# PRBonn/OverlapNet

Hardware: NVIDIA H100
Metric: scan-pairs/sec (overlap+yaw) at 64x900 (higher is better)
Workload: dtype f16

## Files before the change

### overlapnet_b200/csrc/network_tc.cu

```cuda
#include "common.cuh"
#include "hopper.cuh"

#include <cuda_fp16.h>
#include <stddef.h>
#include <stdlib.h>

namespace ovn {

using namespace hopper;

constexpr int WF = 360;
constexpr int CF = 128;
constexpr int S15 = 15;
constexpr int NB = 24;
constexpr int PAIR_ROWS = NB * NB;
constexpr int K4_PITCH = CF;

struct TcState {
  Buffer<__half> w1p;
  Buffer<__half> w2p;
  Buffer<__half> w3p;
  Buffer<float> b2eff;
  Buffer<__half> wres[kMaxLegLayers];
  Buffer<__half> actp[2];
// ... 368 lines not shown
            wgmma_commit();
            if (kk == 1 && sl + 1 < K4_GROUP) rv = *reinterpret_cast<const uint4*>(rp[(sl + 1) & 1] + (sl + 1) * K4_PITCH);
            wgmma_wait<1>();
          }
        wgmma_wait<0>();
        S.w1.release(gi);
      }
      S.right.release(ui);
      if (jb == NB - 1 || u == u_end - 1) S.left.release(pi - 1);
      if (!S.o1s.wait_free(ui)) { atomicExch(err, kErrDeltaO1Consumer); goto done; }
#pragma unroll
      for (int tt = 0; tt < 2; ++tt)
#pragma unroll
        for (int h = 0; h < 2; ++h) {
          if (rows[tt][h] >= blk.rows) continue;
#pragma unroll
          for (int j = 0; j < 8; ++j)
            *reinterpret_cast<uint32_t*>(smem_raw + sto[tt][h][j]) = pack_h2(acc[tt][4 * j + 2 * h], acc[tt][4 * j + 2 * h + 1]);
        }
      fence_proxy_async_smem();
      S.o1s.publish(ui);
    }
  }
done:
  return;
}

constexpr int TC_WG = 2;
constexpr int TC_THREADS = TC_WG * 128 + 32;
constexpr int TC_ROWS = TC_WG * 128;
constexpr uint32_t C2_TILE = 128 * 64 * 2;
constexpr int C2_RING = 3;

struct C2Smem {
  __half A[C2_RING][TC_WG][C2_TILE / 2];
  __half B[C2_RING][2][C2_TILE / 2];
  MbarRing<C2_RING> ring;
};
constexpr size_t C2_SMEM = sizeof(C2Smem) + 1024;
static_assert(C2_SMEM <= 232448, "k_conv2_wgmma shared memory");
static_assert(offsetof(C2Smem, B) % 1024 == 0 && C2_TILE % 1024 == 0, "SWIZZLE_128B tiles on 1024-byte boundaries");

__global__ void __launch_bounds__(TC_THREADS, 1)
k_conv2_wgmma(const __half* __restrict__ o1, const __half* __restrict__ W2s, const float* __restrict__ bias2,
              const float* __restrict__ mu_x3, __half* __restrict__ x3, int64_t out_pitch, int64_t M, int fault,
              int* __restrict__ err) {
  if (fault) {
    if (threadIdx.x == 0 && blockIdx.x == 0) atomicExch(err, kErrInjectedFault);
    return;
  }
  extern __shared__ __align__(128) uint8_t smem_raw[];
  C2Smem& S = *reinterpret_cast<C2Smem*>(smem_raw + ((1024 - (smem_u32(smem_raw) & 1023)) & 1023));
  const int tid = threadIdx.x, warp = tid >> 5, lane = tid & 31;
  const Share tiles = work_share((M + TC_ROWS - 1) / TC_ROWS, blockIdx.x, gridDim.x);
  if (tid == 0) {
    S.ring.init(TC_WG * 4);
    mbar_fence_init();
  }
  __syncthreads();

  if (warp == TC_WG * 4) {
    if (lane == 0) {
      uint32_t gi = 0;
      for (int64_t tile = tiles.begin; tile < tiles.end; ++tile)
        for (int di = 0; di < S15; ++di, ++gi) {
          const uint32_t s = S.ring.slot(gi);
          PIPE_WAIT(S.ring.acquire(gi, 4 * C2_TILE), kErrConv2Producer);
          for (int h = 0; h < TC_WG; ++h)
            bulk_g2s(S.A[s][h], o1 + ((size_t)(tile * TC_WG + h) * S15 + di) * (C2_TILE / 2), C2_TILE, S.ring.bar(gi));
          bulk_g2s(S.B[s], W2s + (size_t)di * C2_TILE, 2 * C2_TILE, S.ring.bar(gi));
        }
    }
  } else {
    const int wg = warp >> 2, wi = warp & 3, g = lane >> 2, t = lane & 3;
    uint32_t gi = 0;
    bool failed = false;
    for (int64_t tile = tiles.begin; tile < tiles.end; ++tile) {
      float acc[2][64];
#pragma unroll
      for (int sub = 0; sub < 2; ++sub)
#pragma unroll
        for (int e = 0; e < 64; ++e) acc[sub][e] = 0.f;
#pragma unroll 1
      for (int di = 0; di < S15; ++di, ++gi) {
        const uint32_t s = S.ring.slot(gi);
        INFLIGHT_WAIT(S.ring.wait(gi), kErrConv2Consumer);
        const uint32_t a_base = smem_u32(S.A[s][wg]), b_base = smem_u32(S.B[s][0]);
        wgmma_fence();
#pragma unroll
        for (int kk = 0; kk < 4; ++kk)
#pragma unroll
          for (int part = 0; part < 2; ++part) {
            const uint64_t bd = desc_kmajor(b_base + part * C2_TILE + kk * 32, 16, 1024, kSwizzle128B);
#pragma unroll
            for (int sub = 0; sub < 2; ++sub)
              wgmma_m64n128k16_ss(acc[sub], desc_kmajor(a_base + sub * (C2_TILE / 2) + kk * 32, 16, 1024, kSwizzle128B), bd);
          }
        wgmma_commit();
        wgmma_wait<1>();
        if (di > 0) S.ring.release(gi - 1);
      }
      wgmma_wait<0>();
      if (failed) goto done;
      S.ring.release(gi - 1);
#pragma unroll
      for (int sub = 0; sub < 2; ++sub)
#pragma unroll
        for (int h = 0; h < 2; ++h) {
          const int64_t m = tile * TC_ROWS + wg * 128 + sub * 64 + wi * 16 + g + 8 * h;
          if (m >= M) continue;
#pragma unroll
          for (int j = 0; j < 16; ++j) {
            const int n = j * 8 + 2 * t;
            const float a = fmaxf(acc[sub][4 * j + 2 * h] + __ldg(bias2 + n), 0.f) - __ldg(mu_x3 + n);
            const float b = fmaxf(acc[sub][4 * j + 2 * h + 1] + __ldg(bias2 + n + 1), 0.f) - __ldg(mu_x3 + n + 1);
            *reinterpret_cast<uint32_t*>(x3 + ((size_t)j * out_pitch + m) * 8 + 2 * t) = pack_h2(a, b);
          }
        }
    }
  }
done:
  return;
}

constexpr int C3_AROWS = TC_ROWS + 2 * NB + 2;
constexpr uint32_t C3_PLANE = C3_AROWS * 16;
constexpr uint32_t C3_SLAB = 4 * 128 * 16;
constexpr int C3_GROUP = 2;
constexpr int C3_NSTAGES = 36 / C3_GROUP;
constexpr int C3_RING = 4;

struct C3Smem {
  __half A[2][16 * C3_PLANE / 2];
  __half B[C3_RING][C3_GROUP * C3_SLAB / 2];
  MbarRing<C3_RING> w3;
  MbarRing<2> x3;
};
static_assert(sizeof(C3Smem) <= 232448, "k_conv3_wgmma shared memory");
static_assert(offsetof(C3Smem, B) % 16 == 0 && C3_PLANE % 16 == 0, "bulk-copy alignment");

__global__ void __launch_bounds__(TC_THREADS, 1)
k_conv3_wgmma(const __half* __restrict__ X3, int64_t a_pitch, const __half* __restrict__ W3p, const float* __restrict__ bias,
              int64_t M, const float* __restrict__ wd, float* __restrict__ partial, int* __restrict__ err) {
  extern __shared__ __align__(128) uint8_t smem_raw[];
  C3Smem& S = *reinterpret_cast<C3Smem*>(smem_raw);
  const int tid = threadIdx.x, warp = tid >> 5, lane = tid & 31;
  const Share tiles = work_share(2 * ((M + TC_ROWS - 1) / TC_ROWS), blockIdx.x, gridDim.x);
  if (tid == 0) {
    S.w3.init(TC_WG * 4);
    S.x3.init(TC_WG * 4);
    mbar_fence_init();
  }
  __syncthreads();

  if (warp == TC_WG * 4) {
    if (lane == 0) {
      const uint32_t nt = (uint32_t)(tiles.end - tiles.begin);
      uint32_t ai = 0, gi = 0;
      for (uint32_t ti = 0; ti < nt; ++ti) {
        const int nh = (int)((tiles.begin + ti) & 1);
        for (int st = 0; st < C3_NSTAGES; ++st, ++gi) {
          while (ai < nt && ai <= ti + 1) {
            if (ai > ti) {
              if (!S.x3.try_acquire(ai, 16 * C3_PLANE)) break;
            } else {
              PIPE_WAIT(S.x3.acquire(ai, 16 * C3_PLANE), kErrConv3X3Producer);
            }
            const int64_t r0 = ((tiles.begin + ai) >> 1) * TC_ROWS;
            for (int pl = 0; pl < 16; ++pl)
              bulk_g2s(S.A[S.x3.slot(ai)] + pl * (C3_PLANE / 2), X3 + ((size_t)pl * a_pitch + r0) * 8, C3_PLANE, S.x3.bar(ai));
            ++ai;
          }
          PIPE_WAIT(S.w3.acquire(gi, C3_GROUP * C3_SLAB), kErrConv3W3Producer);
          bulk_g2s(S.B[S.w3.slot(gi)], W3p + ((size_t)nh * 36 + st * C3_GROUP) * (C3_SLAB / 2), C3_GROUP * C3_SLAB,
                   S.w3.bar(gi));
        }
      }
    }
  } else {
    const int wg = warp >> 2, wi = warp & 3, g = lane >> 2, t = lane & 3;
    const uint32_t b_base = smem_u32(S.B[0]);
    uint32_t gi = 0;
    bool failed = false;
    for (int64_t tile = tiles.begin; tile < tiles.end; ++tile) {
      const uint32_t ti = (uint32_t)(tile - tiles.begin);
      const int nh = (int)(tile & 1);
      const int64_t r0 = (tile >> 1) * TC_ROWS;
      PIPE_WAIT(S.x3.wait(ti), kErrConv3X3Consumer);
      const uint32_t a_rows = smem_u32(S.A[S.x3.slot(ti)]) + wg * 128 * 16;
      float acc[2][64];
#pragma unroll
      for (int sub = 0; sub < 2; ++sub)
#pragma unroll
        for (int e = 0; e < 64; ++e) acc[sub][e] = 0.f;
#pragma unroll 1
      for (int st = 0; st < C3_NSTAGES; ++st, ++gi) {
        const uint32_t s = S.w3.slot(gi);
        INFLIGHT_WAIT(S.w3.wait(gi), kErrConv3W3Consumer);
        wgmma_fence();
#pragma unroll
        for (int sl = 0; sl < C3_GROUP; ++sl) {
          const int slab = st * C3_GROUP + sl, tap = slab >> 2, c32 = slab & 3;
          const uint32_t a_tap = a_rows + ((tap / 3) * NB + tap % 3) * 16;
          const uint32_t slab_addr = b_base + s * (C3_GROUP * C3_SLAB) + sl * C3_SLAB;
#pragma unroll
          for (int kk = 0; kk < 2; ++kk) {
            const int c16 = c32 * 2 + kk;
            const uint64_t bd = desc_kmajor(slab_addr + kk * 4096, 2048, 128, kNoSwizzle);
#pragma unroll
            for (int sub = 0; sub < 2; ++sub)
              wgmma_m64n128k16_ss(acc[sub], desc_kmajor(a_tap + 2 * c16 * C3_PLANE + sub * 64 * 16, C3_PLANE, 128, kNoSwizzle), bd);
          }
        }
        wgmma_commit();
        wgmma_wait<1>();
        if (st > 0) S.w3.release(gi - 1);
      }
      wgmma_wait<0>();
      if (failed) goto done;
      S.w3.release(gi - 1);
      S.x3.release(ti);
#pragma unroll
      for (int sub = 0; sub < 2; ++sub)
#pragma unroll
        for (int h = 0; h < 2; ++h) {
          const int64_t r = r0 + wg * 128 + sub * 64 + wi * 16 + g + 8 * h;
          const int rem = (int)(r % PAIR_ROWS);
          const int yy = rem / NB, xx = rem - yy * NB;
          const bool valid = (r < M) && (yy < NB - 2) && (xx < NB - 2);
          const float* wrow = wd + (size_t)(valid ? (xx * (NB - 2) + yy) : 0) * 256 + nh * 128;
          float sum = 0.f;
#pragma unroll
          for (int j = 0; j < 16; ++j) {
            const int n = j * 8 + 2 * t;
            sum = fmaf(fmaxf(acc[sub][4 * j + 2 * h] + __ldg(bias + nh * 128 + n), 0.f), __ldg(wrow + n), sum);
            sum = fmaf(fmaxf(acc[sub][4 * j + 2 * h + 1] + __ldg(bias + nh * 128 + n + 1), 0.f), __ldg(wrow + n + 1), sum);
          }
          sum += __shfl_xor_sync(0xffffffffu, sum, 1);
          sum += __shfl_xor_sync(0xffffffffu, sum, 2);
          if (t == 0 && r < M) partial[r * 2 + nh] = valid ? sum : 0.f;
        }
    }
  }
done:
  return;
}

constexpr int C6_PARTS = C6_LT * C6_RT;
constexpr int C6_WG = 2;
constexpr int C6_THREADS = C6_WG * 128 + 32;
constexpr int C6_RING = 3;
constexpr int C6_GPITCH = 132;

struct C6Smem {
  __half R[C6_R_BYTES / 2];
  __half L[C6_RING][C6_L_BYTES / 2];
  float G[C6_WG][C6_LROWS * C6_GPITCH];
  MbarRing<C6_RING> left;
  MbarRing<1> right;
};
static_assert(sizeof(C6Smem) <= 232448, "k_corr_wgmma shared memory");
static_assert(offsetof(C6Smem, L) % 16 == 0, "bulk-copy alignment");

__global__ void __launch_bounds__(C6_THREADS, 1)
k_corr_wgmma(const __half* __restrict__ Lc, const int32_t* __restrict__ l_idx, const __half* __restrict__ Rc,
             int r_per_pair, int n_pairs, float* __restrict__ corr_part, int* __restrict__ err) {
  extern __shared__ __align__(128) uint8_t smem_raw[];
  C6Smem& S = *reinterpret_cast<C6Smem*>(smem_raw);
  const int tid = threadIdx.x, warp = tid >> 5, lane = tid & 31;
  const int q = blockIdx.x % C6_RT;
  const Share share = work_share((int64_t)n_pairs * C6_LT, blockIdx.x / C6_RT, gridDim.x / C6_RT);
  const int u_begin = (int)share.begin, u_end = (int)share.end;
  if (tid == 0) {
    S.left.init(4);
    S.right.init(C6_WG * 4);
    mbar_fence_init();
  }
  __syncthreads();

  if (warp == C6_WG * 4) {
    if (lane == 0) {
      uint32_t ri = 0, ui = 0;
      int key = -1;
      for (int u = u_begin; u < u_end; ++u, ++ui) {
        const int p = u / C6_LT, a = u - p * C6_LT;
        if ((r_per_pair ? p : 0) != key) {
          key = r_per_pair ? p : 0;
          PIPE_WAIT(S.right.acquire(ri, C6_R_BYTES), kErrCorrRightProducer);
          bulk_g2s(S.R, Rc + ((size_t)key * C6_RT + q) * (C6_R_BYTES / 2), C6_R_BYTES, S.right.bar(ri));
          ++ri;
        }
        PIPE_WAIT(S.left.acquire(ui, C6_L_BYTES), kErrCorrLeftProducer);
        bulk_g2s(S.L[S.left.slot(ui)], Lc + ((size_t)(l_idx ? l_idx[p] : p) * C6_LT + a) * (C6_L_BYTES / 2), C6_L_BYTES,
                 S.left.bar(ui));
      }
    }
  } else {
    const int wg = warp >> 2, wi = warp & 3, g = lane >> 2, t = lane & 3, tw = tid & 127;
    float* Gw = S.G[wg];
    const uint32_t r_base = smem_u32(S.R);
    uint32_t ri = 0, ui = 0;
    int key = -1;
    bool failed = false;
    for (int u = u_begin; u < u_end; ++u, ++ui) {
      const int p = u / C6_LT, a = u - p * C6_LT;
      if ((r_per_pair ? p : 0) != key) {
        if (key >= 0) S.right.release(ri - 1);
        key = r_per_pair ? p : 0;
        INFLIGHT_WAIT(S.right.wait(ri), kErrCorrRightConsumer);
        ++ri;
      }
      if ((int)(ui & 1) != wg) continue;
      const uint32_t s = S.left.slot(ui);
      INFLIGHT_WAIT(S.left.wait(ui), kErrCorrLeftConsumer);
      const uint32_t l_base = smem_u32(S.L[s]);
      float acc[64];
#pragma unroll
      for (int e = 0; e < 64; ++e) acc[e] = 0.f;
      wgmma_fence();
#pragma unroll
      for (int c16 = 0; c16 < 8; ++c16) {
        const uint64_t ah = desc_kmajor(l_base + c16 * 2 * C6_LROWS * 16, C6_LROWS * 16, 128, kNoSwizzle);
        const uint64_t al = desc_kmajor(l_base + C6_L_BYTES / 2 + c16 * 2 * C6_LROWS * 16, C6_LROWS * 16, 128, kNoSwizzle);
        const uint64_t bh = desc_kmajor(r_base + c16 * 2 * C6_RROWS * 16, C6_RROWS * 16, 128, kNoSwizzle);
        const uint64_t bl = desc_kmajor(r_base + C6_R_BYTES / 2 + c16 * 2 * C6_RROWS * 16, C6_RROWS * 16, 128, kNoSwizzle);
        wgmma_m64n128k16_ss(acc, ah, bh);
        wgmma_m64n128k16_ss(acc, al, bh);
        wgmma_m64n128k16_ss(acc, ah, bl);
      }
      wgmma_commit();
      wgmma_wait<0>();
      S.left.release(ui);
      named_bar_sync(1 + wg, 128);
#pragma unroll
      for (int j = 0; j < 16; ++j) {
        float* r0 = Gw + (wi * 16 + g) * C6_GPITCH + j * 8 + 2 * t;
        *reinterpret_cast<float2*>(r0) = make_float2(acc[4 * j], acc[4 * j + 1]);
        *reinterpret_cast<float2*>(r0 + 8 * C6_GPITCH) = make_float2(acc[4 * j + 2], acc[4 * j + 3]);
      }
      named_bar_sync(1 + wg, 128);
      const int i_lim = min(C6_LROWS, WF - a * C6_LROWS), j_lim = min(C6_RROWS, WF - q * C6_RROWS);
      float* out = corr_part + ((size_t)p * C6_PARTS + a * C6_RT + q) * WF;
      for (int d = tw; d < WF; d += 128) {
        const int dd = d - (C6_RROWS - 1);
        float sum = 0.f;
        if (d < C6_LROWS + C6_RROWS - 1) {
#pragma unroll 8
          for (int ii = 0; ii < C6_LROWS; ++ii) {
            const int jj = ii - dd;
            if (ii < i_lim && jj >= 0 && jj < j_lim) sum += Gw[ii * C6_GPITCH + jj];
          }
        }
        int k = (a * C6_LROWS - q * C6_RROWS + dd - WF / 2) % WF;
        if (k < 0) k += WF;
        out[k] = sum;
      }
    }
  }
done:
  return;
}

template <int EPI>
__global__ void __launch_bounds__(MMA_THREADS)
k_leg_mma(LegArgs g) {
  const int warp = threadIdx.x >> 5, lane = threadIdx.x & 31, gq = lane >> 2, t = lane & 3;
  const int64_t px0 = (int64_t)blockIdx.y * MMA_ROWS + warp * 16;
  if (px0 >= g.M) return;
  const int nz = (g.n_valid + 63) / 64;
  const int y = blockIdx.x, z = blockIdx.z % nz, slice = blockIdx.z / nz;
  const int64_t in_base = (int64_t)(y / g.runs_per_img) * g.in_img_planes + (int64_t)(y % g.runs_per_img) * g.in_run_planes;
  const int64_t pa = px0 + gq < g.M ? px0 + gq : g.M - 1, pb = px0 + gq + 8 < g.M ? px0 + gq + 8 : g.M - 1;
  const int n_slabs = g.kh * g.kw * 3;
  const size_t plane = (size_t)g.a_pitch * 8;
  const int per_tap = g.c8in / 2, n_it = g.kh * g.kw * per_tap;
  const int it0 = n_it * slice / g.n_split, it1 = n_it * (slice + 1) / g.n_split;
  float acc[8][4] = {};
#pragma unroll 1
  for (int it = it0; it < it1;) {
    const int tap = it / per_tap, dh = tap / g.kw, dw = tap - dh * g.kw;
    const int c8_end = (tap + 1) * per_tap < it1 ? g.c8in : (it1 - tap * per_tap) * 2;
    {
      const __half* Ah = g.A + (size_t)(in_base + (int64_t)dh * 2 * g.c8in) * plane + (size_t)dw * 8 + 2 * t;
      const __half* Al = Ah + (size_t)g.c8in * plane;
      const __half* Bh = g.Bp + ((size_t)(z * n_slabs + (dh * g.kw + dw) * 3) * g.c8in * 64 + gq) * 8 + 2 * t;
      const __half* Bl = Bh + (size_t)2 * g.c8in * 64 * 8;
#pragma unroll 1
      for (int c8 = (it - tap * per_tap) * 2; c8 < c8_end; c8 += 2) {
        const size_t o0 = (size_t)c8 * plane, o1 = o0 + plane;
        const uint32_t h0 = ld_h2(Ah + o0 + pa * 8), h1 = ld_h2(Ah + o0 + pb * 8), h2 = ld_h2(Ah + o1 + pa * 8), h3 = ld_h2(Ah + o1 + pb * 8);
        const uint32_t l0 = ld_h2(Al + o0 + pa * 8), l1 = ld_h2(Al + o0 + pb * 8), l2 = ld_h2(Al + o1 + pa * 8), l3 = ld_h2(Al + o1 + pb * 8);
        const size_t bo = (size_t)c8 * 64 * 8;
#pragma unroll
        for (int j = 0; j < 8; ++j) {
          const uint32_t wh0 = ld_h2(Bh + bo + j * 64), wh1 = ld_h2(Bh + bo + 64 * 8 + j * 64);
          const uint32_t wl0 = ld_h2(Bl + bo + j * 64), wl1 = ld_h2(Bl + bo + 64 * 8 + j * 64);
          mma16816(acc[j], h0, h1, h2, h3, wh0, wh1);
          mma16816(acc[j], l0, l1, l2, l3, wh0, wh1);
          mma16816(acc[j], h0, h1, h2, h3, wl0, wl1);
        }
      }
    }
    it = tap * per_tap + c8_end / 2;
  }
#pragma unroll
  for (int h = 0; h < 2; ++h) {
    const int64_t px = px0 + gq + 8 * h;
    if (px >= g.M) continue;
#pragma unroll
    for (int j = 0; j < 8; ++j) {
      const int n = z * 64 + j * 8 + 2 * t;
      if (n >= g.n_valid) continue;
      if (EPI == 5) {
        *reinterpret_cast<float2*>(g.part + (((size_t)slice * gridDim.x + y) * g.M + px) * g.n_valid + n) =
            make_float2(acc[j][2 * h], acc[j][2 * h + 1]);
        continue;
      }
      const float pre_a = acc[j][2 * h] + __ldg(g.bias + n), pre_b = acc[j][2 * h + 1] + __ldg(g.bias + n + 1);
      const float a = fmaxf(pre_a, 0.f), b = fmaxf(pre_b, 0.f);
      if (EPI == 4) {
        if (leg_act_unstorable(pre_a) || leg_act_unstorable(pre_b)) atomicCAS(g.err, 0, kErrNonFiniteOperand);
        const __half2 hi = __floats2half2_rn(a, b);
        const float2 hf = __half22float2(hi);
        const int64_t pl = (int64_t)y * g.out_run_planes + (n >> 3);
        *reinterpret_cast<__half2*>(g.out_planes + ((size_t)pl * g.out_pitch + px) * 8 + (n & 7)) = hi;
        *reinterpret_cast<uint32_t*>(g.out_planes + ((size_t)(pl + g.out_run_planes / 2) * g.out_pitch + px) * 8 + (n & 7)) =
            pack_h2(a - hf.x, b - hf.y);
      } else {
        *reinterpret_cast<float2*>(g.out_f32 + ((size_t)y * g.M + px) * g.n_valid + n) = make_float2(a, b);
      }
    }
  }
}

template <int EPI>
__global__ void __launch_bounds__(256)
k_leg_splitk_reduce(LegArgs g, int rows) {
  const int c8n = g.n_valid / 8;
  const int64_t i = (int64_t)blockIdx.x * blockDim.x + threadIdx.x;
  if (i >= (int64_t)rows * g.M * c8n) return;
  const int c8 = (int)(i % c8n);
  const int64_t px = (i / c8n) % g.M, y = i / c8n / g.M;
  const int64_t slice_stride = (int64_t)rows * g.M * g.n_valid;
  const float* src = g.part + (y * g.M + px) * g.n_valid + c8 * 8;
  float v[8] = {};
  for (int sl = 0; sl < g.n_split; ++sl) {
    const float4 a = __ldg(reinterpret_cast<const float4*>(src + sl * slice_stride));
    const float4 b = __ldg(reinterpret_cast<const float4*>(src + sl * slice_stride + 4));
    v[0] += a.x; v[1] += a.y; v[2] += a.z; v[3] += a.w; v[4] += b.x; v[5] += b.y; v[6] += b.z; v[7] += b.w;
  }
  bool bad = false;
#pragma unroll
  for (int e = 0; e < 8; ++e) {
    v[e] += __ldg(g.bias + c8 * 8 + e);
    bad |= leg_act_unstorable(v[e]);
    v[e] = fmaxf(v[e], 0.f);
  }
  if (EPI == 4) {
    if (bad) atomicCAS(g.err, 0, kErrNonFiniteOperand);
    __half hi[8], lo[8];
#pragma unroll
    for (int e = 0; e < 8; ++e) {
      hi[e] = __float2half_rn(v[e]);
      lo[e] = __float2half_rn(v[e] - __half2float(hi[e]));
    }
    const int64_t pl = y * g.out_run_planes + c8;
    *reinterpret_cast<uint4*>(g.out_planes + ((size_t)pl * g.out_pitch + px) * 8) = *reinterpret_cast<const uint4*>(hi);
    *reinterpret_cast<uint4*>(g.out_planes + ((size_t)(pl + g.out_run_planes / 2) * g.out_pitch + px) * 8) =
        *reinterpret_cast<const uint4*>(lo);
  } else {
    float* dst = g.out_f32 + (y * g.M + px) * g.n_valid + c8 * 8;
    *reinterpret_cast<float4*>(dst) = make_float4(v[0], v[1], v[2], v[3]);
    *reinterpret_cast<float4*>(dst + 4) = make_float4(v[4], v[5], v[6], v[7]);
  }
}

__global__ void __launch_bounds__(384)
k_corr_finalize(const float* __restrict__ part, float* __restrict__ corr_out, int32_t* __restrict__ yaw,
                const int* __restrict__ err) {
  __shared__ float s_corr[WF];
  const int p = blockIdx.x;
  for (int k = threadIdx.x; k < WF; k += blockDim.x) {
    float c = 0.f;
    for (int b = 0; b < C6_PARTS; ++b) c += part[((size_t)p * C6_PARTS + b) * WF + k];
    s_corr[k] = c;
    if (corr_out) corr_out[(size_t)p * WF + k] = c;
  }
  __syncthreads();
  if (threadIdx.x == 0) {
    int best = 0;
    float bv = s_corr[0];
    for (int k = 1; k < WF; ++k)
      if (s_corr[k] > bv) { bv = s_corr[k]; best = k; }
    yaw[p] = (*err != 0) ? INT32_MIN : 180 - best;
  }
}

__global__ void __launch_bounds__(1024)
k_o1_channel_mean(const __half* __restrict__ o1, int64_t M, float* __restrict__ mu) {
  __shared__ float part[16][64];
  const int o = threadIdx.x & 63, g = threadIdx.x >> 6;
  float acc = 0.f;
  for (int64_t m = g; m < M; m += 16)
    for (int di = 0; di < S15; ++di) acc += __half2float(o1[o1_chunk_offset(m, di, o >> 3) + (o & 7)]);
  part[g][o] = acc;
  __syncthreads();
  if (g == 0) {
    float t = 0.f;
    for (int k = 0; k < 16; ++k) t += part[k][o];
    mu[o] = __half2float(__float2half_rn(t / (float)(M * S15)));
  }
}

__global__ void __launch_bounds__(1024)
k_x3_channel_mean(const __half* __restrict__ x3, int64_t pitch, int64_t M, float* __restrict__ mu) {
  __shared__ float part[8][128];
  const int n = threadIdx.x & 127, g = threadIdx.x >> 7;
  float acc = 0.f;
  for (int64_t m = g; m < M; m += 8) acc += __half2float(x3[((size_t)(n >> 3) * pitch + m) * 8 + (n & 7)]);
  part[g][n] = acc;
  __syncthreads();
  if (g == 0) {
    float t = 0.f;
    for (int k = 0; k < 8; ++k) t += part[k][n];
    mu[n] = t / (float)M;
  }
}

__global__ void __launch_bounds__(128)
k_fold_bias2(const float* __restrict__ b2base, const float* __restrict__ mu_o1, const float* __restrict__ W2,
             float* __restrict__ b2eff) {
  const int n = threadIdx.x;
  float acc = b2base[n];
  for (int di = 0; di < S15; ++di)
    for (int o = 0; o < 64; ++o) acc = fmaf(mu_o1[o], W2[((size_t)di * 64 + o) * 128 + n], acc);
  b2eff[n] = acc;
}

__global__ void __launch_bounds__(256)
k_fold_bias3(const float* __restrict__ b3, const float* __restrict__ mu_x3, const float* __restrict__ W3,
             float* __restrict__ b3eff) {
  const int m = threadIdx.x;
  float acc = b3[m];
  for (int tap = 0; tap < 9; ++tap)
    for (int n = 0; n < 128; ++n)
      acc = fmaf(mu_x3[n], W3[((size_t)tap * 128 + n) * 256 + m], acc);
  b3eff[m] = acc;
}

__global__ void __launch_bounds__(256)
k_dense_finalize(const float* __restrict__ partial, const float* __restrict__ bd, int rows_per_pair,
                 float* __restrict__ overlap, const int* __restrict__ err) {
  __shared__ float red[256];
  const int p = blockIdx.x;
  const float* x = partial + (size_t)p * rows_per_pair * 2;
  float acc = 0.f;
  for (int i = threadIdx.x; i < rows_per_pair * 2; i += 256) acc += x[i];
  red[threadIdx.x] = acc;
  __syncthreads();
  for (int o = 128; o > 0; o >>= 1) {
    if (threadIdx.x < o) red[threadIdx.x] += red[threadIdx.x + o];
    __syncthreads();
  }
  if (threadIdx.x == 0) overlap[p] = (*err != 0) ? __int_as_float(0x7fc00000) : 1.0f / (1.0f + expf(-(red[0] + bd[0])));
}

constexpr size_t L1_DIRECT_SMEM = 48 * 1024;
constexpr size_t L1_SMALL_SMEM = 200 * 1024;

template <bool CIN4>
__global__ void __launch_bounds__(512, CIN4 ? 0 : 2)
k_leg_layer1_direct(const float* __restrict__ x, const float* __restrict__ w, const float* __restrict__ bias,
                    int n, int H_in, int W_in, int cin, int kh, int kw, int sh, int sw, int H_out, int W_out,
                    int relu, __half* __restrict__ out, int* __restrict__ err) {
  constexpr int CO = 16;
  extern __shared__ __align__(16) float w_s[];
  const int pairs = (W_out + 1) / 2;
  int64_t idx = (int64_t)blockIdx.x * blockDim.x + threadIdx.x;
  const bool active = idx < (int64_t)n * H_out * pairs;
  if (!active) idx = 0;
  const int xo = 2 * (int)(idx % pairs);
  const int64_t r = idx / pairs;
  const int y = (int)(r % H_out);
  const int64_t img = r / H_out;
  const bool has1 = xo + 1 < W_out;
  float acc0[CO], acc1[CO];
#pragma unroll
  for (int e = 0; e < CO; ++e) acc0[e] = acc1[e] = bias[e];
  const float* base0 = x + ((img * H_in + (int64_t)y * sh) * W_in + (int64_t)xo * sw) * cin;
  const float* base1 = has1 ? base0 + (int64_t)sw * cin : base0;
  for (int dh = 0; dh < kh; ++dh) {
    __syncthreads();
    for (int i = threadIdx.x; i < kw * cin * CO; i += blockDim.x) w_s[i] = w[(size_t)dh * kw * cin * CO + i];
    __syncthreads();
    for (int dw = 0; dw < kw; ++dw) {
      const int64_t off = ((int64_t)dh * W_in + dw) * cin;
      const float* pw = w_s + (size_t)(dw * cin) * CO;
      if (CIN4) {
        const float4 a = __ldg(reinterpret_cast<const float4*>(base0 + off));
        const float4 b = __ldg(reinterpret_cast<const float4*>(base1 + off));
        const float va[4] = {a.x, a.y, a.z, a.w}, vb[4] = {b.x, b.y, b.z, b.w};
#pragma unroll
        for (int c = 0; c < 4; ++c) {
#pragma unroll
          for (int q4 = 0; q4 < 4; ++q4) {
            const float4 wv = *reinterpret_cast<const float4*>(pw + c * CO + q4 * 4);
            acc0[q4 * 4 + 0] = fmaf(va[c], wv.x, acc0[q4 * 4 + 0]); acc1[q4 * 4 + 0] = fmaf(vb[c], wv.x, acc1[q4 * 4 + 0]);
            acc0[q4 * 4 + 1] = fmaf(va[c], wv.y, acc0[q4 * 4 + 1]); acc1[q4 * 4 + 1] = fmaf(vb[c], wv.y, acc1[q4 * 4 + 1]);
            acc0[q4 * 4 + 2] = fmaf(va[c], wv.z, acc0[q4 * 4 + 2]); acc1[q4 * 4 + 2] = fmaf(vb[c], wv.z, acc1[q4 * 4 + 2]);
            acc0[q4 * 4 + 3] = fmaf(va[c], wv.w, acc0[q4 * 4 + 3]); acc1[q4 * 4 + 3] = fmaf(vb[c], wv.w, acc1[q4 * 4 + 3]);
          }
        }
      } else {
        for (int c = 0; c < cin; ++c) {
          const float va = __ldg(base0 + off + c), vb = __ldg(base1 + off + c);
#pragma unroll
          for (int q4 = 0; q4 < 4; ++q4) {
            const float4 wv = *reinterpret_cast<const float4*>(pw + c * CO + q4 * 4);
            acc0[q4 * 4 + 0] = fmaf(va, wv.x, acc0[q4 * 4 + 0]); acc1[q4 * 4 + 0] = fmaf(vb, wv.x, acc1[q4 * 4 + 0]);
            acc0[q4 * 4 + 1] = fmaf(va, wv.y, acc0[q4 * 4 + 1]); acc1[q4 * 4 + 1] = fmaf(vb, wv.y, acc1[q4 * 4 + 1]);
            acc0[q4 * 4 + 2] = fmaf(va, wv.z, acc0[q4 * 4 + 2]); acc1[q4 * 4 + 2] = fmaf(vb, wv.z, acc1[q4 * 4 + 2]);
            acc0[q4 * 4 + 3] = fmaf(va, wv.w, acc0[q4 * 4 + 3]); acc1[q4 * 4 + 3] = fmaf(vb, wv.w, acc1[q4 * 4 + 3]);
          }
        }
      }
    }
  }
  if (!active) return;
#pragma unroll
  for (int p = 0; p < 2; ++p) {
    if (p == 1 && !has1) break;
    const float* acc = p ? acc1 : acc0;
#pragma unroll
    for (int g = 0; g < 2; ++g) {
      __half hi[8], lo[8];
      bool bad = false;
#pragma unroll
      for (int e = 0; e < 8; ++e) {
        const float v = relu ? fmaxf(acc[g * 8 + e], 0.f) : acc[g * 8 + e];
        bad |= leg_act_unstorable(relu ? acc[g * 8 + e] : fabsf(acc[g * 8 + e]));
        hi[e] = __float2half_rn(v);
        lo[e] = __float2half_rn(v - __half2float(hi[e]));
      }
      if (bad) atomicCAS(err, 0, kErrNonFiniteOperand);
      const int64_t plane_hi = r * 4 + g;
      *reinterpret_cast<uint4*>(out + ((size_t)plane_hi * W_out + xo + p) * 8) = *reinterpret_cast<const uint4*>(hi);
      *reinterpret_cast<uint4*>(out + ((size_t)(plane_hi + 2) * W_out + xo + p) * 8) = *reinterpret_cast<const uint4*>(lo);
    }
  }
}

template <bool CIN4>
__global__ void __launch_bounds__(256)
k_leg_layer1_small(const float* __restrict__ x, const float* __restrict__ w, const float* __restrict__ bias,
                    int n, int H_in, int W_in, int cin, int kh, int kw, int sh, int sw, int H_out, int W_out, int cout,
                    int relu, __half* __restrict__ out, int* __restrict__ err) {
  extern __shared__ __align__(16) float w_s[];
  for (int i = threadIdx.x; i < kh * kw * cin * cout; i += blockDim.x) w_s[i] = w[i];
  __syncthreads();
  const int C8 = cout / 8;
  const int64_t idx = (int64_t)blockIdx.x * blockDim.x + threadIdx.x;
  if (idx >= (int64_t)n * H_out * C8 * W_out) return;
  const int xo = (int)(idx % W_out);
  int64_t r = idx / W_out;
  const int g = (int)(r % C8); r /= C8;
  const int y = (int)(r % H_out);
  const int64_t img = r / H_out;
  float acc[8];
#pragma unroll
  for (int e = 0; e < 8; ++e) acc[e] = bias[g * 8 + e];
  const float* base = x + ((img * H_in + (int64_t)y * sh) * W_in + (int64_t)xo * sw) * cin;
  for (int dh = 0; dh < kh; ++dh) {
    for (int dw = 0; dw < kw; ++dw) {
      const float* px = base + ((int64_t)dh * W_in + dw) * cin;
      const float* pw = w_s + (size_t)((dh * kw + dw) * cin) * cout + g * 8;
      if (CIN4) {
        const float4 v = __ldg(reinterpret_cast<const float4*>(px));
        const float vv[4] = {v.x, v.y, v.z, v.w};
#pragma unroll
        for (int c = 0; c < 4; ++c) {
          const float4 w0 = *reinterpret_cast<const float4*>(pw + c * cout);
          const float4 w1 = *reinterpret_cast<const float4*>(pw + c * cout + 4);
          acc[0] = fmaf(vv[c], w0.x, acc[0]); acc[1] = fmaf(vv[c], w0.y, acc[1]);
          acc[2] = fmaf(vv[c], w0.z, acc[2]); acc[3] = fmaf(vv[c], w0.w, acc[3]);
          acc[4] = fmaf(vv[c], w1.x, acc[4]); acc[5] = fmaf(vv[c], w1.y, acc[5]);
          acc[6] = fmaf(vv[c], w1.z, acc[6]); acc[7] = fmaf(vv[c], w1.w, acc[7]);
        }
      } else {
        for (int c = 0; c < cin; ++c) {
          const float vc = __ldg(px + c);
          const float4 w0 = *reinterpret_cast<const float4*>(pw + c * cout);
          const float4 w1 = *reinterpret_cast<const float4*>(pw + c * cout + 4);
          acc[0] = fmaf(vc, w0.x, acc[0]); acc[1] = fmaf(vc, w0.y, acc[1]);
          acc[2] = fmaf(vc, w0.z, acc[2]); acc[3] = fmaf(vc, w0.w, acc[3]);
          acc[4] = fmaf(vc, w1.x, acc[4]); acc[5] = fmaf(vc, w1.y, acc[5]);
          acc[6] = fmaf(vc, w1.z, acc[6]); acc[7] = fmaf(vc, w1.w, acc[7]);
        }
      }
    }
  }
  __half hi[8], lo[8];
  bool bad = false;
#pragma unroll
  for (int e = 0; e < 8; ++e) {
    const float v = relu ? fmaxf(acc[e], 0.f) : acc[e];
    bad |= leg_act_unstorable(relu ? acc[e] : fabsf(acc[e]));
    hi[e] = __float2half_rn(v);
    lo[e] = __float2half_rn(v - __half2float(hi[e]));
  }
  if (bad) atomicCAS(err, 0, kErrNonFiniteOperand);
  const int64_t plane_hi = r * (2 * C8) + g;
  *reinterpret_cast<uint4*>(out + ((size_t)plane_hi * W_out + xo) * 8) = *reinterpret_cast<const uint4*>(hi);
  *reinterpret_cast<uint4*>(out + ((size_t)(plane_hi + C8) * W_out + xo) * 8) = *reinterpret_cast<const uint4*>(lo);
}

static int tc_supported(const ovn_handle* h) {
  return h->net_ok && h->cfg.leg_output_width == WF && h->cfg.conv1size == S15;
}

static int leg_split(const ovn_handle* h, const ConvSpec& L, int n) {
  if (n > 2) return 1;
  const int64_t tiles = (int64_t)n * L.h_out * ((L.w_out + MMA_ROWS - 1) / MMA_ROWS) * ((L.cout + 63) / 64);
  const int64_t n_it = (int64_t)L.kh * L.kw * (L.cin / 16);
  int64_t sp = (4 * h->sm_count + tiles - 1) / tiles;
  if (sp > n_it / 4) sp = n_it / 4;
  return sp < 1 ? 1 : (int)sp;
}

int tc_pack_weights(ovn_handle* h) {
  if (!tc_supported(h))
    OVN_SET_ERR(h, OVN_ERR_BAD_CONFIG, "precision f16_tc supports leg_output_width=360, conv1size=15 only");
  const ConvSpec& L1 = h->leg[0];
  const size_t l1_row_bytes = (size_t)L1.kw * L1.cin * L1.cout * sizeof(float);
  if (L1.cout != 16 || l1_row_bytes > L1_DIRECT_SMEM || l1_row_bytes * L1.kh > L1_SMALL_SMEM)
    OVN_SET_ERR(h, OVN_ERR_BAD_CONFIG, "tensor-core leg: layer %s does not fit k_leg_layer1_direct / _small", L1.name);
  h->tc.reset();
  std::unique_ptr<TcState, TcStateDelete> t(new TcState());
  const LayerWeights& w1 = h->host_w["c_conv1"];
  const LayerWeights& w2 = h->host_w["c_conv2"];
  const LayerWeights& w3 = h->host_w["c_conv3"];
  std::vector<__half> p1((size_t)K4_STEPS * 4 * 64 * 8);
  for (int cc = 0; cc < 4; ++cc)
    for (int dj = 0; dj < S15; ++dj)
      for (int k8 = 0; k8 < 4; ++k8)
        for (int o = 0; o < 64; ++o)
          for (int e = 0; e < 8; ++e) {
            const int c = cc * 32 + k8 * 8 + e;
            p1[((((size_t)(cc * S15 + dj) * 4 + k8) * 64 + o) * 8) + e] =
                __float2half(w1.kernel[((size_t)dj * CF + c) * 64 + o]);
          }
  std::vector<__half> p2((size_t)S15 * 2 * 128 * 64);
  for (int di = 0; di < S15; ++di)
    for (int n = 0; n < 128; ++n)
      for (int o = 0; o < 64; ++o) {
        const float wf = w2.kernel[((size_t)di * 64 + o) * 128 + n];
        const __half wh = __float2half(wf);
        const __half wl = __float2half(wf - __half2float(wh));
        const size_t off = (size_t)n * 64 + (((o >> 3) ^ (n & 7)) << 3) + (o & 7);
        p2[((size_t)di * 2 + 0) * 128 * 64 + off] = wh;
        p2[((size_t)di * 2 + 1) * 128 * 64 + off] = wl;
      }
  std::vector<__half> p3((size_t)2 * 36 * 4 * 128 * 8);
  for (int dy = 0; dy < 3; ++dy)
    for (int dx = 0; dx < 3; ++dx)
      for (int gq = 0; gq < 4; ++gq) {
        const int sl = (dy * 3 + dx) * 4 + gq;
        for (int nh = 0; nh < 2; ++nh)
          for (int j = 0; j < 4; ++j)
            for (int n = 0; n < 128; ++n)
              for (int e = 0; e < 8; ++e) {
                const int c = (gq * 4 + j) * 8 + e;
                p3[((((size_t)nh * 36 + sl) * 4 + j) * 128 + n) * 8 + e] =
                    __float2half(w3.kernel[(((size_t)dx * 3 + dy) * 128 + c) * 256 + nh * 128 + n]);
              }
      }
  std::vector<float> b2e(128);
  {
    const LayerWeights& wb1 = h->host_w["c_conv1"];
    for (int n = 0; n < 128; ++n) {
      double acc = w2.bias[n];
      for (int di = 0; di < S15; ++di)
        for (int o = 0; o < 64; ++o) acc += (double)wb1.bias[o] * (double)w2.kernel[((size_t)di * 64 + o) * 128 + n];
      b2e[n] = (float)acc;
    }
  }
  int rc;
  if ((rc = upload_vec(h, t->b2eff, b2e)) != OVN_OK) return rc;
// ... 424 lines not shown
```

Measured before the change: 213,300.

## Overlap correlation diagonal reduction with next tile's wgmma and skip empty partials

```diff
diff --git a/overlapnet_b200/csrc/network_tc.cu b/overlapnet_b200/csrc/network_tc.cu
--- a/overlapnet_b200/csrc/network_tc.cu
+++ b/overlapnet_b200/csrc/network_tc.cu
@@ -694,6 +694,32 @@
     uint32_t ri = 0, ui = 0;
     int key = -1;
     bool failed = false;
+    const int j_lim = min(C6_RROWS, WF - q * C6_RROWS);
+    auto diagonals = [&](int pp, int aa) {
+      const int i_lim = min(C6_LROWS, WF - aa * C6_LROWS);
+      const int c = tw;
+      const int hi_a = min(c - (C6_RROWS - j_lim), i_lim);
+      const float* ga = Gw + C6_RROWS - c;
+      const float* gb = ga - C6_RROWS;
+      float v[C6_LROWS];
+#pragma unroll
+      for (int ii = 0; ii < C6_LROWS; ++ii) v[ii] = (ii < c ? ga : gb)[ii * (C6_GPITCH + 1)];
+      float sa = 0.f, sb = 0.f;
+#pragma unroll
+      for (int ii = 0; ii < C6_LROWS; ++ii) {
+        if (ii < hi_a) sa += v[ii];
+        if (ii >= c && ii < i_lim) sb += v[ii];
+      }
+      int ka = aa * C6_LROWS - q * C6_RROWS + c - C6_RROWS - WF / 2 + 2 * WF;
+      if (ka >= WF) ka -= WF;
+      if (ka >= WF) ka -= WF;
+      int kb = ka + C6_RROWS;
+      if (kb >= WF) kb -= WF;
+      float* out = corr_part + ((size_t)pp * C6_PARTS + aa * C6_RT + q) * WF;
+      if (c > 0) out[ka] = sa;
+      if (c < C6_LROWS) out[kb] = sb;
+    };
+    int pend_p = -1, pend_a = 0;
     for (int u = u_begin; u < u_end; ++u, ++ui) {
       const int p = u / C6_LT, a = u - p * C6_LT;
       if ((r_per_pair ? p : 0) != key) {
@@ -721,33 +747,27 @@
         wgmma_m64n128k16_ss(acc, ah, bl);
       }
       wgmma_commit();
+      if (pend_p >= 0) diagonals(pend_p, pend_a);
       wgmma_wait<0>();
       S.left.release(ui);
       named_bar_sync(1 + wg, 128);
-#pragma unroll
-      for (int j = 0; j < 16; ++j) {
-        float* r0 = Gw + (wi * 16 + g) * C6_GPITCH + j * 8 + 2 * t;
-        *reinterpret_cast<float2*>(r0) = make_float2(acc[4 * j], acc[4 * j + 1]);
-        *reinterpret_cast<float2*>(r0 + 8 * C6_GPITCH) = make_float2(acc[4 * j + 2], acc[4 * j + 3]);
+      {
+        const int sw = ~g & 1;
+        float* r0 = Gw + (wi * 16 + g) * C6_GPITCH + 2 * t;
+#pragma unroll
+        for (int j = 0; j < 16; ++j)
+#pragma unroll
+          for (int h = 0; h < 2; ++h) {
+            const float x0 = acc[4 * j + 2 * h], x1 = acc[4 * j + 2 * h + 1];
+            r0[h * 8 * C6_GPITCH + j * 8 + sw] = sw ? x1 : x0;
+            r0[h * 8 * C6_GPITCH + j * 8 + 1 - sw] = sw ? x0 : x1;
+          }
       }
       named_bar_sync(1 + wg, 128);
-      const int i_lim = min(C6_LROWS, WF - a * C6_LROWS), j_lim = min(C6_RROWS, WF - q * C6_RROWS);
-      float* out = corr_part + ((size_t)p * C6_PARTS + a * C6_RT + q) * WF;
-      for (int d = tw; d < WF; d += 128) {
-        const int dd = d - (C6_RROWS - 1);
-        float sum = 0.f;
-        if (d < C6_LROWS + C6_RROWS - 1) {
-#pragma unroll 8
-          for (int ii = 0; ii < C6_LROWS; ++ii) {
-            const int jj = ii - dd;
-            if (ii < i_lim && jj >= 0 && jj < j_lim) sum += Gw[ii * C6_GPITCH + jj];
-          }
-        }
-        int k = (a * C6_LROWS - q * C6_RROWS + dd - WF / 2) % WF;
-        if (k < 0) k += WF;
-        out[k] = sum;
-      }
-    }
+      pend_p = p;
+      pend_a = a;
+    }
+    if (pend_p >= 0) diagonals(pend_p, pend_a);
   }
 done:
   return;
@@ -874,7 +894,11 @@
   const int p = blockIdx.x;
   for (int k = threadIdx.x; k < WF; k += blockDim.x) {
     float c = 0.f;
-    for (int b = 0; b < C6_PARTS; ++b) c += part[((size_t)p * C6_PARTS + b) * WF + k];
+    for (int b = 0; b < C6_PARTS; ++b) {
+      const int a = b / C6_RT, q = b - a * C6_RT;
+      const int d = (k - a * C6_LROWS + q * C6_RROWS + C6_RROWS - 1 + WF / 2 + WF) % WF;
+      if (d < C6_LROWS + C6_RROWS - 1) c += part[((size_t)p * C6_PARTS + b) * WF + k];
+    }
     s_corr[k] = c;
     if (corr_out) corr_out[(size_t)p * WF + k] = c;
   }
```

Result: no change. 218,000, median of 6 (+2.2%).
